# Chriz122/ultralytics_pro

Measured on AMD Instinct MI355X. Metric: images/sec (whole job = n_gpus x per-GPU bs=32) YOLOv8n 640x640 (forward + Detect decode + NMS), higher is better.
Workload: dtype bf16

## Files before the change

include/upa.h:

```cpp
#ifndef UPA_H
#define UPA_H
#include <stddef.h>
#include <stdint.h>

#ifdef __cplusplus
extern "C" {
#endif

enum { UPA_F32 = 0, UPA_BF16 = 1, UPA_U8_BGR_HWC = 2  };
enum { UPA_ACT_NONE = 0, UPA_ACT_SILU = 1, UPA_ACT_RELU = 2 };
enum { UPA_OK = 0, UPA_EINVAL = -1, UPA_EUNSUPPORTED = -2, UPA_EWORKSPACE = -3, UPA_ELAUNCH = -4 };

typedef struct upa_opts {
  uint32_t size;
  int32_t conv_big;
  int32_t conv_big_bm;
  int32_t conv_ckt;
  int32_t no_ws, no_pipe, no_1x1, no_c16, no_upcat;
  int32_t pipe_all;
  int32_t pipe_min_tiles;
  int32_t pipe_wgs, c16_wgs;
  int32_t c1_mt, c1_waves, c1_wgs;
  int32_t pair;
  int32_t pair_tile64, pair_tile32;
  int32_t no_pair_cv2;
  int32_t c2f;
  int32_t c2f16_waves;
  int32_t c2f32_th;
  int32_t no_branch_tail;
  int32_t branch_tail_bm;
  int32_t stem_wgs, stemf_wgs, stemf_waves, stem_no_mfma;
  int32_t ablate_conv, ablate_pipe, ablate_c1, ablate_stem;
  int32_t c2f64_max_px;
  int32_t conv_ws3;
  int32_t no_group;
  int32_t no_c2f32_up;
  int32_t no_xcd;
  int32_t keys_only;
  int32_t conv_p8;
  int32_t c2f_stream;
  int32_t c2f_stream_rows;
  int32_t no_stack_first;
  int32_t no_epi_stats;
  int32_t nms_stages;
  int32_t nms_first_prefix;
  int32_t detect_stream;
  int32_t detect_stream_rows;
  int32_t no_sppf_front;
  int32_t no_c2f16_down;
} upa_opts;

int upa_version(void);
const char* upa_last_error(void);
size_t upa_opts_size(void);

size_t upa_conv_packed_weight_bytes(int cout, int cin, int k, int dtype);
int upa_pack_conv_weight(const float* w_oihw, int cout, int cin, int k, int dtype, void* out);
int upa_conv2d_bias_act(const void* x, int n, int h, int w, int cin, int ldx,
                        const void* w_packed, const float* bias ,
                        void* y, int cout, int ldy,
                        const void* residual , int ldr,
                        int k, int stride, int pad, int act, int dtype, const upa_opts* opts, void* stream);
typedef struct upa_conv_problem {
  const void* x; int32_t n, h, w, cin, ldx;
  const void* w_packed; const float* bias;
  void* y; int32_t cout, ldy;
  const void* residual; int32_t ldr;
} upa_conv_problem;
int upa_conv2d_bias_act_group(const upa_conv_problem* probs, int count, int k, int stride, int pad, int act, int dtype,
                              const upa_opts* opts, void* stream);

int upa_conv2d_pool2(const void* x, int n, int h, int w, int cin, int ldx, const void* w_packed, const float* bias, void* y, int cout,
                     int ldy, int k, int stride, int pad, int act, int dtype, const upa_opts* opts, void* stream);
int upa_conv2d_stem_nchw_pool2(const void* x_nchw, int x_dtype, int n, int cin, int h, int w, const float* w_oihw, const float* bias,
                               void* y, int cout, int ldy, int k, int stride, int pad, int act, int dtype, const upa_opts* opts,
                               void* stream);

int upa_conv_variant(int n, int h, int w, int cin, int cout, int k, int stride, int pad, int dtype, const upa_opts* opts);

int upa_bottleneck_pair(const void* x, int n, int h, int w, int c, int ldx, const void* w1_packed, const float* b1,
                        const void* w2_packed, const float* b2, void* y, int ldy, int residual, int act, int dtype,
                        const upa_opts* opts, void* stream);
int upa_bottleneck_pair_e(const void* x, int n, int h, int w, int c, int cmid, int ldx, const void* w1_packed, const float* b1,
                          const void* w2_packed, const float* b2, void* y, int ldy, int residual, int act, int dtype,
                          const upa_opts* opts, void* stream);


size_t upa_stem_packed_weight_bytes(int cout, int cin, int k);
int upa_pack_stem_weight(const float* w_oihw, int cout, int cin, int k, float* out );
int upa_conv2d_stem_nchw(const void* x_nchw, int x_dtype, int n, int cin, int h, int w,
                         const float* w_oihw, const float* bias, void* y, int cout, int ldy,
                         int k, int stride, int pad, int act, int dtype, const upa_opts* opts, void* stream);

int upa_stem_conv_fused(const void* x, int n, int h, int w, const float* w0, const float* b0, const void* w1,
                        const float* b1, void* y, int ldy, const upa_opts* opts, void* stream);
int upa_stem_conv_fused_k(const void* x, int n, int h, int w, int k0, const float* w0, const float* b0, const void* w1,
                          const float* b1, void* y, int ldy, const upa_opts* opts, void* stream);
int upa_stem_conv_fused_c(const void* x, int n, int h, int w, int k0, int c0, const float* w0, const float* b0, const void* w1,
                          const float* b1, void* y, int ldy, const upa_opts* opts, void* stream);
int upa_stem_conv_fused_s(const void* x, int n, int h, int w, int k0, int s0, int c0, const float* w0, const float* b0,
                          const void* w1, const float* b1, void* y, int ldy, const upa_opts* opts, void* stream);

// ... 227 lines not shown
```

ultralytics_pro_amd/_lib.py:

```python

from __future__ import annotations

import ctypes as C
import os
from pathlib import Path

import torch

UPA_F32, UPA_BF16, UPA_U8_BGR_HWC = 0, 1, 2
UPA_EUNSUPPORTED = -2
ACT_NONE, ACT_SILU, ACT_RELU = 0, 1, 2

_PKG = Path(__file__).resolve().parent
LIB_PATH = Path(os.environ.get("UPA_HIP_LIB", _PKG / "libupa_hip.so"))

_vp, _i, _f, _sz = C.c_void_p, C.c_int, C.c_float, C.c_size_t


class Opts(C.Structure):

    _fields_ = [("size", C.c_uint32), ("conv_big", _i), ("conv_big_bm", _i), ("conv_ckt", _i),
                ("no_ws", _i), ("no_pipe", _i), ("no_1x1", _i), ("no_c16", _i), ("no_upcat", _i),
                ("pipe_all", _i), ("pipe_min_tiles", _i), ("pipe_wgs", _i), ("c16_wgs", _i),
                ("c1_mt", _i), ("c1_waves", _i), ("c1_wgs", _i),
                ("pair", _i), ("pair_tile64", _i), ("pair_tile32", _i), ("no_pair_cv2", _i),
                ("c2f", _i), ("c2f16_waves", _i), ("c2f32_th", _i),
                ("no_branch_tail", _i), ("branch_tail_bm", _i),
                ("stem_wgs", _i), ("stemf_wgs", _i), ("stemf_waves", _i), ("stem_no_mfma", _i),
                ("ablate_conv", _i), ("ablate_pipe", _i), ("ablate_c1", _i), ("ablate_stem", _i), ("c2f64_max_px", _i), ("conv_ws3", _i), ("no_group", _i), ("no_c2f32_up", _i), ("no_xcd", _i), ("keys_only", _i), ("conv_p8", _i), ("c2f_stream", _i), ("c2f_stream_rows", _i), ("no_stack_first", _i), ("no_epi_stats", _i), ("nms_stages", _i), ("nms_first_prefix", _i), ("detect_stream", _i), ("detect_stream_rows", _i), ("no_sppf_front", _i), ("no_c2f16_down", _i)]

    def __init__(self, **kw):
        super().__init__()
        self.size = C.sizeof(Opts)
        for k, v in kw.items():
            if k in dict(self._fields_):
                setattr(self, k, int(v))
            else:
                raise AttributeError(f"upa_opts has no field '{k}'")

    def replace(self, **kw) -> "Opts":
        o = Opts()
        C.memmove(C.byref(o), C.byref(self), C.sizeof(Opts))
        for k, v in kw.items():
            setattr(o, k, int(v))
        return o

    _ENV = {"UPA_CONV_BIG": ("conv_big", lambda v: {0: 1, 1: 0, 2: 2}[int(v)]), "UPA_CONV_BIG_BM": ("conv_big_bm", int), "UPA_CONV_WS3": ("conv_ws3", int),
            "UPA_CONV_CKT": ("conv_ckt", int), "UPA_CONV_NO_WS": ("no_ws", lambda v: 1), "UPA_CONV_NO_PIPE": ("no_pipe", lambda v: 1),
            "UPA_CONV_NO_1X1": ("no_1x1", lambda v: 1), "UPA_CONV_NO_C16": ("no_c16", lambda v: 1), "UPA_NO_UPCAT": ("no_upcat", lambda v: 1),
            "UPA_PIPE_ALL": ("pipe_all", lambda v: 1), "UPA_PIPE_MIN_TILES": ("pipe_min_tiles", int), "UPA_PIPE_WGS": ("pipe_wgs", int),
            "UPA_C16_WGS": ("c16_wgs", int), "UPA_C1_MT": ("c1_mt", int), "UPA_C1_WAVES": ("c1_waves", int), "UPA_C1_WGS": ("c1_wgs", int),
            "UPA_NO_PAIR": ("pair", lambda v: {0: 2, 1: 1, 2: 0, 3: 3}[int(v)]), "UPA_PAIR_T64": ("pair_tile64", int),
            "UPA_PAIR_T32": ("pair_tile32", int), "UPA_NO_PAIR_CV2": ("no_pair_cv2", int), "UPA_NO_C2F": ("c2f", int),
            "UPA_C2F16_WAVES": ("c2f16_waves", int), "UPA_C2F32_TH": ("c2f32_th", int), "UPA_NO_BRANCH_TAIL": ("no_branch_tail", int),
            "UPA_BRANCH_TAIL_BM": ("branch_tail_bm", int), "UPA_STEM_WGS": ("stem_wgs", int), "UPA_STEMF_WGS": ("stemf_wgs", int),
            "UPA_STEMF_WAVES": ("stemf_waves", int), "UPA_STEM_NO_MFMA": ("stem_no_mfma", lambda v: 1),
            "UPA_CONV_ABLATE": ("ablate_conv", int), "UPA_PIPE_ABLATE": ("ablate_pipe", int), "UPA_C1_ABLATE": ("ablate_c1", int),
            "UPA_STEM_ABLATE": ("ablate_stem", int)}

    @classmethod
    def from_env(cls, env=None) -> "Opts":
        env = os.environ if env is None else env
        o = cls()
        for name, (field, conv) in cls._ENV.items():
            if name in env:
                setattr(o, field, conv(env[name]))
        return o


class BranchLevel(C.Structure):
    _fields_ = [("x", C.c_void_p), ("n", _i), ("h", _i), ("w", _i), ("c", _i), ("ldx", _i), ("w3_packed", C.c_void_p), ("b3", C.c_void_p),
                ("wt_packed", C.c_void_p), ("bt", C.c_void_p), ("stride_px", C.c_float), ("a0", _i)]


class DetectBranch(C.Structure):
    _fields_ = [("c", _i), ("reserved", _i), ("w1", C.c_void_p), ("b1", C.c_void_p), ("w2", C.c_void_p), ("b2", C.c_void_p),
                ("wt", C.c_void_p), ("bt", C.c_void_p)]


class ConvProblem(C.Structure):
    _fields_ = [("x", C.c_void_p), ("n", _i), ("h", _i), ("w", _i), ("cin", _i), ("ldx", _i), ("w_packed", C.c_void_p), ("bias", C.c_void_p),
                ("y", C.c_void_p), ("cout", _i), ("ldy", _i), ("residual", C.c_void_p), ("ldr", _i)]
# ... 169 lines not shown
```

ultralytics_pro_amd/csrc/conv_big.hip:

```cpp
#include <stdlib.h>

#include <mutex>
#include <type_traits>
#include <unordered_map>

#include "common.h"
#include "conv_pipe.h"
UPA_STAMP_DEFINE(conv_big)

template <int KS, int STRIDE, int WM, int WN, int MT, int NT, int TAIL = 0>
__device__ __forceinline__ void conv_big_body(const BigParams& p, const int bid0) {
  static_assert(WM * WN == 8, "8 waves per workgroup");
  static_assert(TAIL == 0 || TAIL == 3 || TAIL == 4 || WN == 1, "a tail needs every channel of a pixel in one wave");
  static_assert(TAIL != 1 || (NT % 2) == 0, "box branch: 64 channels");
  static_assert(TAIL != 3 || (NT % 2) == 0, "the statistics epilogue pairs n-tiles");
  static_assert(TAIL != 4 || ((NT % 2) == 0 && KS == 2 && STRIDE == 1), "the interleaving epilogue: 2 x 2 phase kernels, paired n-tiles");
  constexpr int NTB = WN * NT;
  constexpr int WBUF = 2 * NTB * 1024;
  extern __shared__ __attribute__((aligned(16))) char smem[];
  const int tid = threadIdx.x;
  const int lane = tid & 63;
  const int wave = __builtin_amdgcn_readfirstlane(tid >> 6);
  const int r = lane & 15, g = lane >> 4;
  const int wm = wave / WN, wn = wave % WN;

  const int tilesPerImg = p.tilesX * p.tilesY;
  int bid = p.no_xcd ? bid0 : upa_xcd_tile(bid0, tilesPerImg * p.N);
  const int n = bid / tilesPerImg;
  bid -= n * tilesPerImg;
  const int tyi = bid / p.tilesX;
  const int txi = bid - tyi * p.tilesX;
  const int oy0 = tyi * p.TH, ox0 = txi * p.TW;
  const int iy0 = oy0 * STRIDE - p.pad, ix0 = ox0 * STRIDE - p.pad;
  const int ntb0 = blockIdx.y * NTB;

  const int haloItems = p.IH * p.IWp * 8;
  const int haloPadded = (haloItems + 63) & ~63;
  char* hal = smem;
  char* wbuf = smem + (size_t)haloPadded * 16;

  int pl0[MT], pty[MT], ptx[MT];
#pragma unroll
  for (int i = 0; i < MT; ++i) {
    const int pp = (wm * MT + i) * 16 + r;
    int ty = (int)__umulhi((unsigned)pp, p.magicTW);
    int tx = pp - ty * p.TW;
    if (ty >= p.TH) { ty = p.TH; tx = 0; }
    pty[i] = ty;
    ptx[i] = tx;
    pl0[i] = ty < p.TH ? (ty * STRIDE) * p.IWp + tx : 0;
  }

  f32x4 acc[MT][NT];
#pragma unroll
  for (int i = 0; i < MT; ++i)
#pragma unroll
    for (int j = 0; j < NT; ++j) acc[i][j] = f32x4{0.f, 0.f, 0.f, 0.f};

  constexpr int TAPS = KS * KS;
  const int nChunks = (p.KTT + 1) >> 1;

  auto stage_halo = [&](int c) __attribute__((always_inline)) {
    const int c0 = c * 64;
    for (int base = wave * 64; base < haloPadded; base += 512) {
      const int idx = base + lane;
      const int pix = idx >> 3;
      const int slot = idx & 7;
      const int cg = slot ^ (pix & 7);
      const int py = (int)__umulhi((unsigned)pix, p.magicIW);
      const int qx = pix - py * p.IWp;
      int px = qx;
      if constexpr (STRIDE == 2) px = qx < p.HALF ? 2 * qx : 2 * (qx - p.HALF) + 1;
      const int iy = iy0 + py, ix = ix0 + px;
      const int ch = c0 + cg * 8;
      const char* src = reinterpret_cast<const char*>(g_zero16);
      if (idx < haloItems && px < p.IW && iy >= 0 && iy < p.H && ix >= 0 && ix < p.W && ch < p.Cin)
        src = p.x + ((((size_t)n * p.H + iy) * p.W + ix) * (size_t)p.ldx + ch) * 2;
      lds_dma16(src, hal + base * 16);
    }
  };
  auto stage_w = [&](int c, int tap, int b) __attribute__((always_inline)) {
#pragma unroll
    for (int f0 = 0; f0 < 2 * NTB; f0 += 8) {
      const int f = f0 + wave;
      if (f < 2 * NTB) {
        const int kt = f / NTB, j = f - kt * NTB;
        const int ktg = c * 2 + kt;
        const int nt = ntb0 + j;
        const char* src = reinterpret_cast<const char*>(g_zero16);
        if (ktg < p.KTT && nt < p.NTn) src = p.w + (((size_t)(tap * p.KTT + ktg) * p.NTn + nt) * 64 + lane) * 16;
        lds_dma16(src, wbuf + b * WBUF + f * 1024);
      }
    }
  };

  UPA_STAMP_AT(0);
  UPA_STAMP_HWID();
  stage_halo(0);
  stage_w(0, 0, 0);
  int buf = 0;
  for (int c = 0; c < nChunks; ++c) {
    int kh = 0, kw = 0;
#pragma unroll 1
    for (int tap = 0; tap < TAPS; ++tap) {
      asm volatile("s_waitcnt vmcnt(0)" ::: "memory");
      __syncthreads();
      if (c == 0) UPA_STAMP_AT(1 + tap);
      if (tap + 1 < TAPS) stage_w(c, tap + 1, buf ^ 1);
      const int tapshift = kh * p.IWp + (STRIDE == 2 ? (kw >> 1) + (kw & 1) * p.HALF : kw);
      const char* wb = wbuf + buf * WBUF + (wn * NT) * 1024 + lane * 16;
      int paddr[MT], pswz[MT];
#pragma unroll
      for (int i = 0; i < MT; ++i) {
        const int pl = pl0[i] + tapshift;
        paddr[i] = pl * 128;
        pswz[i] = pl & 7;
      }
#pragma unroll
      for (int kt = 0; kt < 2; ++kt) {
        if constexpr (TAIL == 2) {
          if (kt == 1 && c * 2 + 1 >= p.KTT) break;
        }
        if constexpr (NT <= 6) {
          u32x4 a[NT], b[MT];
#pragma unroll
          for (int j = 0; j < NT; ++j) a[j] = *reinterpret_cast<const u32x4*>(wb + (kt * NTB + j) * 1024);
#pragma unroll
          for (int i = 0; i < MT; ++i) b[i] = *reinterpret_cast<const u32x4*>(hal + paddr[i] + (((kt * 4 + g) ^ pswz[i]) << 4));
#pragma unroll
          for (int i = 0; i < MT; ++i)
#pragma unroll
            for (int j = 0; j < NT; ++j)
              acc[i][j] = __builtin_amdgcn_mfma_f32_16x16x32_bf16(*reinterpret_cast<const bf16x8*>(&a[j]),
                                                                  *reinterpret_cast<const bf16x8*>(&b[i]), acc[i][j], 0, 0, 0);
        } else {
          constexpr int GS = (NT + 1) / 2;
          u32x4 b[MT];
#pragma unroll
          for (int i = 0; i < MT; ++i) b[i] = *reinterpret_cast<const u32x4*>(hal + paddr[i] + (((kt * 4 + g) ^ pswz[i]) << 4));
#pragma unroll
          for (int j0 = 0; j0 < NT; j0 += GS) {
            u32x4 a[GS];
#pragma unroll
            for (int j = 0; j < GS; ++j)
              if (j0 + j < NT) a[j] = *reinterpret_cast<const u32x4*>(wb + (kt * NTB + j0 + j) * 1024);
#pragma unroll
            for (int i = 0; i < MT; ++i)
#pragma unroll
              for (int j = 0; j < GS; ++j)
                if (j0 + j < NT)
                  acc[i][j0 + j] = __builtin_amdgcn_mfma_f32_16x16x32_bf16(*reinterpret_cast<const bf16x8*>(&a[j]),
                                                                           *reinterpret_cast<const bf16x8*>(&b[i]), acc[i][j0 + j], 0, 0, 0);
            __builtin_amdgcn_sched_barrier(0);
          }
        }
      }
      buf ^= 1;
      if (++kw == KS) { kw = 0; ++kh; }
    }
    if (c + 1 < nChunks) {
      __syncthreads();
      stage_halo(c + 1);
      stage_w(c + 1, 0, buf);
    }
  }
  UPA_STAMP_AT(10);

  if constexpr (TAIL == 1 || TAIL == 2) {
    f32x4 bv[NT];
#pragma unroll
    for (int j = 0; j < NT; ++j) bv[j] = *reinterpret_cast<const f32x4*>(p.bias + j * 16 + g * 4);
    f32x4 acc2[MT][NT];
#pragma unroll
    for (int i = 0; i < MT; ++i)
#pragma unroll
      for (int j = 0; j < NT; ++j) acc2[i][j] = f32x4{0.f, 0.f, 0.f, 0.f};
#pragma unroll
    for (int s2 = 0; s2 < NT / 2; ++s2) {
      u32x4 hb[MT];
#pragma unroll
      for (int i = 0; i < MT; ++i) {
        float v0[4], v1[4];
#pragma unroll
        for (int q = 0; q < 4; ++q) {
          v0[q] = act_rcp<UPA_ACT_SILU>(acc[i][2 * s2][q] + bv[2 * s2][q]);
          v1[q] = act_rcp<UPA_ACT_SILU>(acc[i][2 * s2 + 1][q] + bv[2 * s2 + 1][q]);
        }
        hb[i] = u32x4{pack_bf16x2(v0[0], v0[1]), pack_bf16x2(v0[2], v0[3]), pack_bf16x2(v1[0], v1[1]), pack_bf16x2(v1[2], v1[3])};
      }
#pragma unroll
      for (int j = 0; j < NT; ++j) {
        const u32x4 a2 = *reinterpret_cast<const u32x4*>(p.tw + ((size_t)(s2 * NT + j) * 64 + lane) * 16);
#pragma unroll
        for (int i = 0; i < MT; ++i)
          acc2[i][j] = __builtin_amdgcn_mfma_f32_16x16x32_bf16(*reinterpret_cast<const bf16x8*>(&a2),
                                                               *reinterpret_cast<const bf16x8*>(&hb[i]), acc2[i][j], 0, 0, 0);
      }
    }
    if constexpr (NT & 1) {
      typedef __attribute__((ext_vector_type(4))) short s16x4;
      constexpr int j0 = NT - 1, s2 = NT / 2;
      u32x2 hh[MT];
#pragma unroll
      for (int i = 0; i < MT; ++i) {
        float v0[4];
#pragma unroll
        for (int q = 0; q < 4; ++q) v0[q] = act_rcp<UPA_ACT_SILU>(acc[i][j0][q] + bv[j0][q]);
        hh[i] = u32x2{pack_bf16x2(v0[0], v0[1]), pack_bf16x2(v0[2], v0[3])};
      }
#pragma unroll
      for (int j = 0; j < NT; ++j) {
        const u32x2 a2 = *reinterpret_cast<const u32x2*>(p.tw + ((size_t)(s2 * NT + j) * 64 + lane) * 16);
#pragma unroll
        for (int i = 0; i < MT; ++i)
          acc2[i][j] = __builtin_amdgcn_mfma_f32_16x16x16bf16_1k(*reinterpret_cast<const s16x4*>(&a2),
                                                                 *reinterpret_cast<const s16x4*>(&hh[i]), acc2[i][j], 0, 0, 0);
// ... 181 lines not shown
  else if (p.act == UPA_ACT_RELU) epilogue(std::integral_constant<int, UPA_ACT_RELU>{});
  else epilogue(std::integral_constant<int, UPA_ACT_NONE>{});
  UPA_STAMP_AT(11);
#ifdef UPA_STAMP
  asm volatile("s_waitcnt vmcnt(0)" ::: "memory");
  UPA_STAMP_AT(12);
#endif
}

template <int KS, int STRIDE, int WM, int WN, int MT, int NT, int TAIL = 0>
__global__ __launch_bounds__(512, 4) void conv_big_kernel(const BigParams p) {
  conv_big_body<KS, STRIDE, WM, WN, MT, NT, TAIL>(p, (int)blockIdx.x);
}

template <int KS, int STRIDE, int WM, int WN, int MT, int NT, int TAIL = 0>
__global__ __launch_bounds__(512, 4) void conv_big_pair_kernel(const BigParams p0, const BigParams p1, const int split) {
  if ((int)blockIdx.x < split) conv_big_body<KS, STRIDE, WM, WN, MT, NT, TAIL>(p0, (int)blockIdx.x);
  else conv_big_body<KS, STRIDE, WM, WN, MT, NT, TAIL>(p1, (int)blockIdx.x - split);
}
template <int KS, int STRIDE, int WM, int WN, int MT, int NT, int TAIL = 0>
__global__ __launch_bounds__(512, 4) void conv_big_tri_kernel(const BigParams p0, const BigParams p1, const BigParams p2, const int s0,
                                                              const int s1) {
  if ((int)blockIdx.x < s0) conv_big_body<KS, STRIDE, WM, WN, MT, NT, TAIL>(p0, (int)blockIdx.x);
  else if ((int)blockIdx.x < s1) conv_big_body<KS, STRIDE, WM, WN, MT, NT, TAIL>(p1, (int)blockIdx.x - s0);
  else conv_big_body<KS, STRIDE, WM, WN, MT, NT, TAIL>(p2, (int)blockIdx.x - s1);
}

template <int KS_, int STRIDE_, int WM_, int WN_, int MT_, int NT_, int TAIL_>
struct BigCfg {
  static constexpr int NTB = WN_ * NT_;
  __device__ static __forceinline__ void run(const BigParams& p, int bid) { conv_big_body<KS_, STRIDE_, WM_, WN_, MT_, NT_, TAIL_>(p, bid); }
};
template <class CA, class CB>
__global__ __launch_bounds__(512, 4) void conv_big_mix_kernel(const BigParams a0, const BigParams a1, const BigParams b0, const BigParams b1,
                                                              const int s0, const int s1, const int s2) {
  const int b = (int)blockIdx.x;
  if (b < s0) CA::run(a0, b);
  else if (b < s1) CA::run(a1, b - s0);
  else if (b < s2) CB::run(b0, b - s1);
  else CB::run(b1, b - s2);
}

namespace {
void big_halo_geometry(BigParams& p, bool tight = false) {
  p.IH = (p.TH - 1) * p.stride + p.KS;
  p.IW = (p.TW - 1) * p.stride + p.KS;
  p.HALF = p.stride == 2 ? (p.IW + 1) / 2 : 0;
  const int minp = p.stride == 2 ? 2 * p.HALF : p.IW;
  p.IWp = tight ? minp : upa_lds_pick_pitch(minp, p.TW, p.TH * p.TW, p.stride);
  p.magicTW = (unsigned)((0x100000000ULL + p.TW - 1) / p.TW);
  p.magicIW = (unsigned)((0x100000000ULL + p.IWp - 1) / p.IWp);
}
size_t big_halo_bytes(const BigParams& p) { return (((size_t)p.IH * p.IWp * 8 + 63) & ~(size_t)63) * 16; }

bool big_pick_tile(BigParams& p, int bm, int ntb, size_t lds_cap) {
  struct Pick { int th, tw, tight; };
  static std::mutex mu;
  static std::unordered_map<unsigned long long, Pick> memo;
  const unsigned long long key = ((unsigned long long)p.OH << 48) ^ ((unsigned long long)p.OW << 32) ^ ((unsigned long long)bm << 20) ^
                                 ((unsigned long long)ntb << 12) ^ ((unsigned long long)(lds_cap >> 9) << 3) ^ ((unsigned long long)p.KS << 56) ^ (p.KS == 3 ? 4u : 0u) ^
                                 (p.stride == 2 ? 2u : 0u);
  {
    std::lock_guard<std::mutex> lk(mu);
    auto it = memo.find(key);
    if (it != memo.end()) {
      if (it->second.th <= 0) return false;
      p.TH = it->second.th; p.TW = it->second.tw;
      big_halo_geometry(p, it->second.tight != 0);
      return true;
    }
  }
  long best = -1;
  int bth = 0, btw = 0;
  bool btight = false;
  for (int tw = 2; tw <= 256 && tw <= ((p.OW + 1) & ~1); ++tw) {
    int th0 = bm / tw;
    if (th0 > p.OH) th0 = p.OH;
    if (th0 < 1) continue;
    const int thb = cdiv(p.OH, cdiv(p.OH, th0));
    for (int pass = 0; pass < 2; ++pass) {
      const int th = pass ? thb : th0;
      if (pass && thb == th0) break;
      for (int tight = 0; tight < 2; ++tight) {
        p.TH = th; p.TW = tw;
        big_halo_geometry(p, tight != 0);
        const size_t lds = big_halo_bytes(p) + 2 * (size_t)(2 * ntb * 1024) + 256;
        if (lds > lds_cap) continue;
        const long tiles = (long)cdiv(p.OW, tw) * cdiv(p.OH, th);
        const long cost = tiles * 65536 + (long)p.IH * p.IWp;
        if (best < 0 || cost < best) { best = cost; bth = th; btw = tw; btight = tight != 0; }
        break;
      }
    }
  }
  p.TH = bth; p.TW = btw;
  if (best >= 0) big_halo_geometry(p, btight);
  {
    std::lock_guard<std::mutex> lk(mu);
    memo[key] = Pick{best >= 0 ? bth : 0, btw, btight ? 1 : 0};
  }
  return best >= 0;
}

template <int KS, int STRIDE, int WM, int WN, int MT, int NT, int TAIL = 0>
int big_launch_inst(const BigParams& p, size_t lds, hipStream_t s) {
  constexpr int NTB = WN * NT;
// ... 76 lines not shown
  return (unsigned short)(u >> 16);
}

extern "C" int upa_pack_tail_weight(const float* w, int cout, int cin, void* out) {
  UPA_CHECK_ARG(w && out && cout > 0 && cin > 0, "pack_tail_weight: bad args");
  const int ks = cdiv(cin, 32), nt = cdiv(cout, 16);
  unsigned short* o = (unsigned short*)out;
  size_t idx = 0;
  for (int s = 0; s < ks; ++s)
    for (int j = 0; j < nt; ++j)
      for (int lane = 0; lane < 64; ++lane) {
        const int g = lane >> 4, r = lane & 15;
        const int co = 16 * j + r;
        for (int e = 0; e < 8; ++e, ++idx) {
          const int ci = 32 * s + (e < 4 ? 4 * g + e : 16 + 4 * g + e - 4);
          o[idx] = big_host_bf16((co < cout && ci < cin) ? w[(size_t)co * cin + ci] : 0.f);
        }
      }
  return UPA_OK;
}

namespace {
int branch_tail_prepare(BigParams& p, int& ntb, int& bm, size_t& lds, const void* x, int n, int h, int w, int c, int ldx,
                        const void* w3_packed, const float* b3, const void* wt_packed, const float* bt, int kind, int nc,
                        float stride_px, float* y, int a_total, int a0, unsigned long long* best_keys, int dtype, const upa_opts* opts) {
  UPA_CHECK_ARG(x && w3_packed && b3 && wt_packed && bt && y, "detect_branch_tail: null pointer");
  UPA_CHECK_ARG(kind == 1 || kind == 2, "detect_branch_tail: kind must be 1 (box) or 2 (class)");
  UPA_CHECK_ARG(n > 0 && h > 0 && w > 0 && a0 >= 0 && a0 + h * w <= a_total, "detect_branch_tail: level does not fit a_total");
  const int off = UPA_OPT(opts, no_branch_tail);
  ntb = kind == 1 ? 4 : (c == 80 ? 5 : 6);
  if (off || dtype != UPA_BF16 || c % 8 != 0 || ldx % 8 != 0 || h * w < 2 || w < 2 || (kind == 1 && c != 64) ||
      (kind == 2 && (c > 96 || nc > ntb * 16)) || ((uintptr_t)x % 16) != 0 || !upa_magic_exact((long)h * w - 1, w)) {
    upa_set_error("detect_branch_tail: outside the fused form (bf16; box c = 64; class c <= 96, nc <= 96)");
    return UPA_EUNSUPPORTED;
  }
  memset(&p, 0, sizeof(p));
  p.x = (const char*)x; p.w = (const char*)w3_packed; p.bias = b3; p.tw = (const char*)wt_packed; p.tb = bt;
  p.N = n; p.H = h; p.W = w; p.Cin = c; p.ldx = ldx; p.OH = h; p.OW = w; p.Cout = ntb * 16; p.KS = 3; p.stride = 1; p.pad = 1;
  p.act = UPA_ACT_SILU;
  p.KTT = cdiv(c, 32);
  p.NTn = ntb;
  p.de.y = y; p.de.a_total = a_total; p.de.a0 = a0; p.de.HW = h * w; p.de.W = w;
  p.de.magicHW = upa_magic_div(h * w); p.de.magicW = upa_magic_div(w);
  p.de.nc = nc; p.de.stride_px = stride_px;
  if (kind == 2 && best_keys && (long)a_total * nc < (1L << 31)) p.de.best_keys = best_keys;
  p.de.keys_only = (p.de.best_keys && UPA_OPT(opts, keys_only)) ? 1 : 0;
  p.no_xcd = UPA_OPT(opts, no_xcd);
  const long px = (long)n * h * w;
  bm = (px + 255) / 256 < upa_num_cus() ? 128 : 256;
  if (const int f = UPA_OPT(opts, branch_tail_bm); f == 128 || f == 256) bm = f;
  if (!big_pick_tile(p, bm, ntb, 80 * 1024 - 512) && !big_pick_tile(p, bm, ntb, 160 * 1024)) return UPA_EUNSUPPORTED;
  p.tilesX = cdiv(p.OW, p.TW);
  p.tilesY = cdiv(p.OH, p.TH);
  lds = big_halo_bytes(p) + 2 * (size_t)(2 * ntb * 1024) + 256;
  return UPA_OK;
}
int branch_tail_launch(const BigParams& p, int kind, int ntb, int bm, size_t lds, hipStream_t s) {
  if (kind == 1) return bm == 256 ? big_launch_inst<3, 1, 8, 1, 2, 4, 1>(p, lds, s) : big_launch_inst<3, 1, 8, 1, 1, 4, 1>(p, lds, s);
  if (ntb == 5) return bm == 256 ? big_launch_inst<3, 1, 8, 1, 2, 5, 2>(p, lds, s) : big_launch_inst<3, 1, 8, 1, 1, 5, 2>(p, lds, s);
  return bm == 256 ? big_launch_inst<3, 1, 8, 1, 2, 6, 2>(p, lds, s) : big_launch_inst<3, 1, 8, 1, 1, 6, 2>(p, lds, s);
}
}

extern "C" int upa_detect_branch_tail(const void* x, int n, int h, int w, int c, int ldx, const void* w3_packed, const float* b3,
                                      const void* wt_packed, const float* bt, int kind, int nc, float stride_px, float* y,
                                      int a_total, int a0, unsigned long long* best_keys, int dtype, const upa_opts* opts,
                                      void* stream) {
  BigParams p;
  int ntb = 0, bm = 0;
  size_t lds = 0;
  if (const int rc = branch_tail_prepare(p, ntb, bm, lds, x, n, h, w, c, ldx, w3_packed, b3, wt_packed, bt, kind, nc, stride_px, y,
                                         a_total, a0, best_keys, dtype, opts); rc != UPA_OK)
    return rc;
  return branch_tail_launch(p, kind, ntb, bm, lds, (hipStream_t)stream);
}

extern "C" int upa_detect_branch_tail_group(const upa_branch_level* levels, int count, int kind, int nc, float* y, int a_total,
                                            unsigned long long* best_keys, int dtype, const upa_opts* opts, void* stream) {
  UPA_CHECK_ARG(levels && count >= 1 && count <= 8, "detect_branch_tail_group: 1..8 levels");
  BigParams ps[8];
  int ntb[8], bm[8];
  size_t lds[8];
  for (int i = 0; i < count; ++i) {
    const upa_branch_level& v = levels[i];
    if (const int rc = branch_tail_prepare(ps[i], ntb[i], bm[i], lds[i], v.x, v.n, v.h, v.w, v.c, v.ldx, v.w3_packed, v.b3, v.wt_packed,
                                           v.bt, kind, nc, v.stride_px, y, a_total, v.a0, best_keys, dtype, opts); rc != UPA_OK)
      return rc;
  }
  hipStream_t s = (hipStream_t)stream;
  const int grouping = UPA_OPT(opts, no_group);
  auto max3 = [](size_t a, size_t b, size_t c) { return a > b ? (a > c ? a : c) : (b > c ? b : c); };
  for (int i = 0; i < count;) {
    if (grouping == 2 && i + 2 < count && ntb[i] == ntb[i + 1] && ntb[i] == ntb[i + 2] && ntb[i] != 6 && bm[i + 1] == 128 && bm[i + 2] == 128) {
      BigParams p0 = ps[i];
      int ntb0 = ntb[i], bm0 = bm[i];
      size_t lds0 = lds[i];
      int rc = UPA_OK;
      if (bm0 != 128) {
        upa_opts o;
        memset(&o, 0, sizeof(o));
        if (opts) memcpy(&o, opts, opts->size < sizeof(o) ? opts->size : sizeof(o));
        o.size = sizeof(o);
        o.branch_tail_bm = 128;
        const upa_branch_level& v = levels[i];
        rc = branch_tail_prepare(p0, ntb0, bm0, lds0, v.x, v.n, v.h, v.w, v.c, v.ldx, v.w3_packed, v.b3, v.wt_packed, v.bt, kind, nc,
                                 v.stride_px, y, a_total, v.a0, best_keys, dtype, &o);
      }
// ... 63 lines not shown
  return UPA_OK;
}

bool upa_conv_big_pick_tile(BigParams& p, int bm, int ntb, size_t lds_cap) { return big_pick_tile(p, bm, ntb, lds_cap); }

bool upa_conv_big_eligible(const ConvShape& s, const upa_opts* opts) {
  const int mode = UPA_OPT(opts, conv_big);
  if (mode == 1) return false;
  const int k = s.k, stride = s.stride, cin = s.cin, cout = s.cout;
  if (s.dtype != UPA_BF16 || !((k == 1 && stride == 1) || (k == 2 && stride == 1) || (k == 3 && (stride == 1 || stride == 2))) || s.pad != k / 2) return false;
  if (cin % 8 != 0 || s.ldx % 8 != 0 || cout % 8 != 0 || s.ldy % 8 != 0 || s.ldr % 8 != 0) return false;
  if (s.act != UPA_ACT_SILU && s.act != UPA_ACT_NONE && s.act != UPA_ACT_RELU) return false;
  if (mode == 2) return cout >= 64;
  const int oh = (s.h + 2 * s.pad - k) / stride + 1, ow = (s.w + 2 * s.pad - k) / stride + 1;
  const long px = (long)s.n * oh * ow;
  if (k == 1) {
    if (cout % 128 != 0 || px < 2048) return false;
    if (cout >= 1024 && cin >= 128 && px >= 32 * 1024) return true;
    return cin >= 512 && !upa_conv1x1_eligible(s, opts);
  }
  if (cin < 64 || px < 2048) return false;
  if (cout % 128 == 0) return cin >= 128 || (px >= 8192 && (stride == 2 || px >= 200 * 1024));
  if (px < 8192) return false;
  if (cout == 80 || cout == 96) return stride == 1 && k == 3;
  if (cout == 144) return stride == 1 && k == 3;
  if (cout == 64) return stride == 1;
  return false;
}

namespace {
int big_prepare(BigParams& p, int& ntb, int& bm, size_t& lds, const upa_opts* opts, bool query_only, int force_ntb = 0) {
  p.KTT = (p.Cin + 31) / 32;
  p.NTn = (p.Cout + 15) / 16;
  ntb = p.NTn <= 4 ? 4 : (p.NTn <= 6 ? 6 : 8);
  if (p.NTn == 5 && p.KS == 3 && p.stride == 1) ntb = 5;
  if (p.NTn == 9 && p.KS == 3 && p.stride == 1) ntb = 9;
  if (force_ntb == 5 && p.NTn <= 5 && p.KS == 3 && p.stride == 1) ntb = 5;
  const long px = (long)p.N * p.OH * p.OW;
  if (ntb == 8 && p.NTn % 4 == 0 && (px + 127) / 128 * cdiv(p.NTn, 8) < upa_num_cus()) ntb = 4;
  const int cols = cdiv(p.NTn, ntb);
  bm = 256;
  if ((px + 255) / 256 * cols < upa_num_cus()) bm = 128;
  if (const int f = UPA_OPT(opts, conv_big_bm); f == 128 || f == 256 || (f == 512 && p.KS == 3 && p.stride == 1 && (ntb == 4 || ntb == 5))) bm = f;
  if (query_only) return UPA_OK;
  if (p.KS == 1) {
    p.N = 1; p.H = 1; p.W = (int)px; p.OH = 1; p.OW = (int)px;
    p.TH = 1; p.TW = bm;
    big_halo_geometry(p, true);
  } else if (!big_pick_tile(p, bm, ntb, 80 * 1024 - 512) && !big_pick_tile(p, bm, ntb, 160 * 1024)) {
    return UPA_EUNSUPPORTED;
  }
  p.tilesX = cdiv(p.OW, p.TW);
  p.tilesY = cdiv(p.OH, p.TH);
  lds = big_halo_bytes(p) + 2 * (size_t)(2 * ntb * 1024) + 256;
  if (lds > 160 * 1024) return UPA_EUNSUPPORTED;
  return UPA_OK;
}
template <int WM, int WN, int MT, int NT>
int big_launch_ks_stats(const BigParams& p, size_t lds, hipStream_t s) {
  if (p.KS == 1) return big_launch_inst<1, 1, WM, WN, MT, NT, 3>(p, lds, s);
  if (p.KS != 3) return UPA_EUNSUPPORTED;
  if (p.stride == 2) return big_launch_inst<3, 2, WM, WN, MT, NT, 3>(p, lds, s);
  return big_launch_inst<3, 1, WM, WN, MT, NT, 3>(p, lds, s);
}
int big_dispatch_stats(const BigParams& p, int ntb, int bm, size_t lds, hipStream_t s) {
  if (bm != 128 && bm != 256) return UPA_EUNSUPPORTED;
  if (ntb == 8) return bm == 256 ? big_launch_ks_stats<4, 2, 4, 4>(p, lds, s) : big_launch_ks_stats<4, 2, 2, 4>(p, lds, s);
  if (ntb == 4) return bm == 256 ? big_launch_ks_stats<8, 1, 2, 4>(p, lds, s) : big_launch_ks_stats<4, 2, 2, 2>(p, lds, s);
  return UPA_EUNSUPPORTED;
}
int big_dispatch(const BigParams& p, int ntb, int bm, size_t lds, hipStream_t s) {
  if (bm == 512) return ntb == 5 ? big_launch_inst<3, 1, 8, 1, 4, 5>(p, lds, s) : big_launch_inst<3, 1, 8, 1, 4, 4>(p, lds, s);
  if (ntb == 5) return bm == 256 ? big_launch_inst<3, 1, 8, 1, 2, 5>(p, lds, s) : big_launch_inst<3, 1, 8, 1, 1, 5>(p, lds, s);
  if (ntb == 9) return bm == 256 ? big_launch_inst<3, 1, 8, 1, 2, 9>(p, lds, s) : big_launch_inst<3, 1, 8, 1, 1, 9>(p, lds, s);
  if (ntb == 8) return bm == 256 ? big_launch_ks<4, 2, 4, 4>(p, lds, s) : big_launch_ks<4, 2, 2, 4>(p, lds, s);
  if (ntb == 6) return bm == 256 ? big_launch_ks<4, 2, 4, 3>(p, lds, s) : big_launch_ks<4, 2, 2, 3>(p, lds, s);
  return bm == 256 ? big_launch_ks<8, 1, 2, 4>(p, lds, s) : big_launch_ks<4, 2, 2, 2>(p, lds, s);
}
}

int upa_conv_big_launch(BigParams p, int query_only, int* variant, void* stream, const upa_opts* opts) {
  p.no_xcd = UPA_OPT(opts, no_xcd);
  int ntb = 0, bm = 0;
  size_t lds = 0;
  const int rc = big_prepare(p, ntb, bm, lds, opts, query_only != 0);
  if (variant) *variant = (1 << 23) | (ntb << 4) | (bm >> 7);
  if (query_only || rc != UPA_OK) return rc;
  return big_dispatch(p, ntb, bm, lds, (hipStream_t)stream);
}

int upa_conv_big_launch_interleave(BigParams p, void* stream, const upa_opts* opts) {
  p.no_xcd = UPA_OPT(opts, no_xcd);
  if (p.KS != 2 || p.stride != 1 || p.act != UPA_ACT_NONE || p.bias || p.il_c % 8 != 0 || p.Cout != 4 * p.il_c) return UPA_EUNSUPPORTED;
  int ntb = 0, bm = 0;
  size_t lds = 0;
  if (const int rc = big_prepare(p, ntb, bm, lds, opts, false); rc != UPA_OK) return rc;
  if (ntb != 8 || (bm != 128 && bm != 256)) return UPA_EUNSUPPORTED;
  hipStream_t s = (hipStream_t)stream;
  return bm == 256 ? big_launch_inst<2, 1, 4, 2, 4, 4, 4>(p, lds, s) : big_launch_inst<2, 1, 4, 2, 2, 4, 4>(p, lds, s);
}

int upa_conv_big_launch_stats(BigParams p, int* rows, long max_rows, void* stream, const upa_opts* opts) {
  p.no_xcd = UPA_OPT(opts, no_xcd);
  if (!p.stats || p.res || p.act != UPA_ACT_NONE) return UPA_EUNSUPPORTED;
  int ntb = 0, bm = 0;
  size_t lds = 0;
  if (const int rc = big_prepare(p, ntb, bm, lds, opts, false); rc != UPA_OK) return rc;
// ... 81 lines not shown
```

ultralytics_pro_amd/csrc/conv_pipe.h:

```cpp
#pragma once
struct ConvShape {
  int n, h, w, cin, ldx, cout, ldy, ldr, k, stride, pad, act, dtype;
};
struct PipeParams {
  const char* x;
  char* y;
  const char* res;
  const char* w;
  const float* bias;
  int N, H, W, Cin, ldx, Cout, ldy, ldr;
  int KTT, NTn, nt0;
  int tilesX, tilesY, numTiles;
  int act;
  int pool;
#ifdef UPA_ABLATE
  int ablate;
#endif
};
bool upa_conv_pipe_eligible(const ConvShape& s, const upa_opts* opts);
int upa_conv_pipe_launch(PipeParams p, int query_only, int* variant, void* stream, const upa_opts* opts);

#include "detect_epi.h"
struct C1Params {
  const char* x;
  char* y;
  const char* w;
  const float* bias;
  int P;
  int Cin, ldx, Cout, ldy;
  int KTT, NTn, groups;
  int act;
#ifdef UPA_ABLATE
  int ablate;
#endif
  int epi;
  DetectEpi de;
  float* stats;
  int stats_ld;
  const char* up;
  int upKT, up_ld, upH, upW;
  unsigned upMagicW, upMagicH;
};
bool upa_conv1x1_eligible(const ConvShape& s, const upa_opts* opts);
int upa_conv1x1_launch(C1Params p, int n_pixels, int query_only, int* variant, void* stream, const upa_opts* opts);
int upa_conv1x1_launch_stats(C1Params p, int n_pixels, int* rows, long max_rows, void* stream, const upa_opts* opts);

struct BigParams {
  const char* x;
  char* y;
  const char* res;
  const char* w;
  const float* bias;
  int N, H, W, Cin, ldx, OH, OW, Cout, ldy, ldr;
  int KS, stride, pad;
  int TH, TW, tilesX, tilesY, IH, IW;
  int IWp;
  int HALF;
  int KTT, NTn;
  int act;
  unsigned magicTW, magicIW;
  int no_xcd;
  const char* tw;
  const float* tb;
  DetectEpi de;
  float* stats;
  int stats_ld;
  int il_h, il_w, il_c;
};
bool upa_conv_big_eligible(const ConvShape& s, const upa_opts* opts);
int upa_conv_big_launch(BigParams p, int query_only, int* variant, void* stream, const upa_opts* opts);
int upa_conv_big_launch_stats(BigParams p, int* rows, long max_rows, void* stream, const upa_opts* opts);
int upa_conv_big_launch_interleave(BigParams p, void* stream, const upa_opts* opts);
int upa_conv_big_launch_group(const BigParams* probs, int count, int* consumed, void* stream, const upa_opts* opts);

bool upa_conv_big_pick_tile(BigParams& p, int bm, int ntb, size_t lds_cap);

bool upa_conv_p8_eligible(const ConvShape& s, const upa_opts* opts);
int upa_conv_p8_launch(BigParams p, int query_only, int* variant, void* stream, const upa_opts* opts);

bool upa_conv_ws3_eligible(const ConvShape& s, const upa_opts* opts);
int upa_conv_ws3_launch(BigParams p, int query_only, int* variant, void* stream, const upa_opts* opts);
int upa_conv_ws3_launch_stats(BigParams p, int* rows, long max_rows, void* stream, const upa_opts* opts);

struct PairParams {
  const char* x;
  char* y;
  const char* w1;
  const char* w2;
  const float* b1;
  const float* b2;
  int N, H, W, OH, OW, ldx, ldy;
  int TH, TW, tilesX, tilesY;
  int IWp, MWp;
  unsigned magicIW, magicMW, magicTW;
  const char* y0;
  const char* wc_std;
  const char* wc_b;
  const float* bc;
  char* out; int ldout;
};
```

Before: 61100.

## Add opt-in cross-chunk halo prefetch and multi-stage LDS ring to big conv

Adds a double-buffered halo for conv kernels with KS>1. The next channel chunk's halo is staged piece by piece during the current chunk's taps, with partial vmcnt waits. Adds a 2–3 stage LDS ring for 1x1 kernels with BM=128, so that halo and weight loads for later chunks overlap MFMA work. The aim is to remove the full-drain barrier and serial halo reload between chunks, at the cost of more LDS per workgroup and possibly lower occupancy. Both paths are chosen through a new no_chunk_prefetch option, and the default value appears to keep the old plain layout.

```diff
diff --git a/include/upa.h b/include/upa.h
--- a/include/upa.h
+++ b/include/upa.h
@@ -48,6 +48,7 @@
   int32_t detect_stream_rows;
   int32_t no_sppf_front;
   int32_t no_c2f16_down;
+  int32_t no_chunk_prefetch;
 } upa_opts;
 
 int upa_version(void);
diff --git a/ultralytics_pro_amd/_lib.py b/ultralytics_pro_amd/_lib.py
--- a/ultralytics_pro_amd/_lib.py
+++ b/ultralytics_pro_amd/_lib.py
@@ -27,7 +27,8 @@
                 ("c2f", _i), ("c2f16_waves", _i), ("c2f32_th", _i),
                 ("no_branch_tail", _i), ("branch_tail_bm", _i),
                 ("stem_wgs", _i), ("stemf_wgs", _i), ("stemf_waves", _i), ("stem_no_mfma", _i),
-                ("ablate_conv", _i), ("ablate_pipe", _i), ("ablate_c1", _i), ("ablate_stem", _i), ("c2f64_max_px", _i), ("conv_ws3", _i), ("no_group", _i), ("no_c2f32_up", _i), ("no_xcd", _i), ("keys_only", _i), ("conv_p8", _i), ("c2f_stream", _i), ("c2f_stream_rows", _i), ("no_stack_first", _i), ("no_epi_stats", _i), ("nms_stages", _i), ("nms_first_prefix", _i), ("detect_stream", _i), ("detect_stream_rows", _i), ("no_sppf_front", _i), ("no_c2f16_down", _i)]
+                ("ablate_conv", _i), ("ablate_pipe", _i), ("ablate_c1", _i), ("ablate_stem", _i), ("c2f64_max_px", _i), ("conv_ws3", _i), ("no_group", _i), ("no_c2f32_up", _i), ("no_xcd", _i), ("keys_only", _i), ("conv_p8", _i), ("c2f_stream", _i), ("c2f_stream_rows", _i), ("no_stack_first", _i), ("no_epi_stats", _i), ("nms_stages", _i), ("nms_first_prefix", _i), ("detect_stream", _i), ("detect_stream_rows", _i), ("no_sppf_front", _i), ("no_c2f16_down", _i),
+                ("no_chunk_prefetch", _i)]
 
     def __init__(self, **kw):
         super().__init__()
diff --git a/ultralytics_pro_amd/csrc/conv_big.hip b/ultralytics_pro_amd/csrc/conv_big.hip
--- a/ultralytics_pro_amd/csrc/conv_big.hip
+++ b/ultralytics_pro_amd/csrc/conv_big.hip
@@ -7,6 +7,33 @@
 #include "common.h"
 #include "conv_pipe.h"
 UPA_STAMP_DEFINE(conv_big)
+
+namespace {
+template <int N>
+__device__ __forceinline__ void big_vm_wait_imm() {
+  static_assert(N >= 0 && N < 64, "vmcnt is a 6-bit field");
+  asm volatile("s_waitcnt vmcnt(%0)" ::"n"(N) : "memory");
+}
+template <int NS>
+__device__ __forceinline__ void big_vm_wait_stages(const int young) {
+  if (young == 1) big_vm_wait_imm<NS>();
+  else if (young == 2) big_vm_wait_imm<2 * NS>();
+  else big_vm_wait_imm<0>();
+}
+__device__ __forceinline__ void big_vm_wait_piece(const int n) {
+  if (n == 1) big_vm_wait_imm<1>();
+  else if (n == 2) big_vm_wait_imm<2>();
+  else if (n == 3) big_vm_wait_imm<3>();
+  else big_vm_wait_imm<0>();
+}
+__device__ __forceinline__ void big_barrier() {
+  __builtin_amdgcn_sched_barrier(0);
+  asm volatile("s_waitcnt lgkmcnt(0)" ::: "memory");
+  __builtin_amdgcn_s_barrier();
+  asm volatile("" ::: "memory");
+  __builtin_amdgcn_sched_barrier(0);
+}
+}
 
 template <int KS, int STRIDE, int WM, int WN, int MT, int NT, int TAIL = 0>
 __device__ __forceinline__ void conv_big_body(const BigParams& p, const int bid0) {
@@ -36,8 +63,11 @@
 
   const int haloItems = p.IH * p.IWp * 8;
   const int haloPadded = (haloItems + 63) & ~63;
-  char* hal = smem;
-  char* wbuf = smem + (size_t)haloPadded * 16;
+  const int HB = haloPadded * 16;
+  constexpr int BM = WM * MT * 16;
+  constexpr bool RING_OK = KS == 1 && BM == 128, HALO2_OK = KS > 1 && BM <= 256;
+  const bool halo2 = HALO2_OK && p.halo2 != 0;
+  char* wbuf = smem + (halo2 ? 2 * HB : HB);
 
   int pl0[MT], pty[MT], ptx[MT];
 #pragma unroll
@@ -60,9 +90,11 @@
   constexpr int TAPS = KS * KS;
   const int nChunks = (p.KTT + 1) >> 1;
 
-  auto stage_halo = [&](int c) __attribute__((always_inline)) {
+  auto stage_halo = [&](int c, char* dst, int k0, int kstep) __attribute__((always_inline)) {
     const int c0 = c * 64;
-    for (int base = wave * 64; base < haloPadded; base += 512) {
+    int issued = 0;
+    for (int base = wave * 64 + k0 * 512; base < haloPadded; base += kstep * 512) {
+      ++issued;
       const int idx = base + lane;
       const int pix = idx >> 3;
       const int slot = idx & 7;
@@ -76,10 +108,11 @@
       const char* src = reinterpret_cast<const char*>(g_zero16);
       if (idx < haloItems && px < p.IW && iy >= 0 && iy < p.H && ix >= 0 && ix < p.W && ch < p.Cin)
         src = p.x + ((((size_t)n * p.H + iy) * p.W + ix) * (size_t)p.ldx + ch) * 2;
-      lds_dma16(src, hal + base * 16);
-    }
+      lds_dma16(src, dst + base * 16);
+    }
+    return issued;
   };
-  auto stage_w = [&](int c, int tap, int b) __attribute__((always_inline)) {
+  auto stage_w = [&](int c, int tap, char* dst) __attribute__((always_inline)) {
 #pragma unroll
     for (int f0 = 0; f0 < 2 * NTB; f0 += 8) {
       const int f = f0 + wave;
@@ -89,79 +122,129 @@
         const int nt = ntb0 + j;
         const char* src = reinterpret_cast<const char*>(g_zero16);
         if (ktg < p.KTT && nt < p.NTn) src = p.w + (((size_t)(tap * p.KTT + ktg) * p.NTn + nt) * 64 + lane) * 16;
-        lds_dma16(src, wbuf + b * WBUF + f * 1024);
+        lds_dma16(src, dst + f * 1024);
+      }
+    }
+  };
+
+  auto mma_tap = [&](const char* hb, const char* wslab, const int tapshift, const int c) __attribute__((always_inline)) {
+    const char* wb = wslab + (wn * NT) * 1024 + lane * 16;
+    int paddr[MT], pswz[MT];
+#pragma unroll
+    for (int i = 0; i < MT; ++i) {
+      const int pl = pl0[i] + tapshift;
+      paddr[i] = pl * 128;
+      pswz[i] = pl & 7;
+    }
+#pragma unroll
+    for (int kt = 0; kt < 2; ++kt) {
+      if constexpr (TAIL == 2) {
+        if (kt == 1 && c * 2 + 1 >= p.KTT) break;
+      }
+      if constexpr (NT <= 6) {
+        u32x4 a[NT], b[MT];
+#pragma unroll
+        for (int j = 0; j < NT; ++j) a[j] = *reinterpret_cast<const u32x4*>(wb + (kt * NTB + j) * 1024);
+#pragma unroll
+        for (int i = 0; i < MT; ++i) b[i] = *reinterpret_cast<const u32x4*>(hb + paddr[i] + (((kt * 4 + g) ^ pswz[i]) << 4));
+#pragma unroll
+        for (int i = 0; i < MT; ++i)
+#pragma unroll
+          for (int j = 0; j < NT; ++j)
+            acc[i][j] = __builtin_amdgcn_mfma_f32_16x16x32_bf16(*reinterpret_cast<const bf16x8*>(&a[j]),
+                                                                *reinterpret_cast<const bf16x8*>(&b[i]), acc[i][j], 0, 0, 0);
+      } else {
+        constexpr int GS = (NT + 1) / 2;
+        u32x4 b[MT];
+#pragma unroll
+        for (int i = 0; i < MT; ++i) b[i] = *reinterpret_cast<const u32x4*>(hb + paddr[i] + (((kt * 4 + g) ^ pswz[i]) << 4));
+#pragma unroll
+        for (int j0 = 0; j0 < NT; j0 += GS) {
+          u32x4 a[GS];
+#pragma unroll
+          for (int j = 0; j < GS; ++j)
+            if (j0 + j < NT) a[j] = *reinterpret_cast<const u32x4*>(wb + (kt * NTB + j0 + j) * 1024);
+#pragma unroll
+          for (int i = 0; i < MT; ++i)
+#pragma unroll
+            for (int j = 0; j < GS; ++j)
+              if (j0 + j < NT)
+                acc[i][j0 + j] = __builtin_amdgcn_mfma_f32_16x16x32_bf16(*reinterpret_cast<const bf16x8*>(&a[j]),
+                                                                         *reinterpret_cast<const bf16x8*>(&b[i]), acc[i][j0 + j], 0, 0, 0);
+          __builtin_amdgcn_sched_barrier(0);
+        }
       }
     }
   };
 
   UPA_STAMP_AT(0);
   UPA_STAMP_HWID();
-  stage_halo(0);
-  stage_w(0, 0, 0);
-  int buf = 0;
-  for (int c = 0; c < nChunks; ++c) {
-    int kh = 0, kw = 0;
+  bool ringed = false;
+  if constexpr (RING_OK) {
+    if (p.ring >= 2) {
+      ringed = true;
+      constexpr int HPW = WM * MT / 4;
+      constexpr int NWLO = (2 * NTB) / 8, NWHI = (2 * NTB + 7) / 8;
+      const int nw = (2 * NTB - wave + 7) >> 3;
+      const int D = p.ring;
+      const int STG = HB + WBUF;
+      auto stage = [&](int c, char* dst) __attribute__((always_inline)) {
+#pragma unroll
+        for (int k = 0; k < HPW; ++k) stage_halo(c, dst, k, HPW);
+        stage_w(c, 0, dst + HB);
+      };
+      for (int d = 0; d < D; ++d) stage(d, smem + d * STG);
+      char* cur = smem;
+      char* prev = smem;
+      for (int c = 0; c < nChunks; ++c) {
+        int young = D - 1;
+        if (c > 0) young = (c + D - 2 < nChunks - 1 ? c + D - 2 : nChunks - 1) - c;
+        if (NWLO == NWHI || nw == NWHI) big_vm_wait_stages<HPW + NWHI>(young);
+        else big_vm_wait_stages<HPW + NWLO>(young);
+        big_barrier();
+        if (c < 9) UPA_STAMP_AT(1 + c);
+        if (c > 0 && c + D - 1 < nChunks) stage(c + D - 1, prev);
+        mma_tap(cur, cur + HB, 0, c);
+        prev = cur;
+        cur += STG;
+        if (cur == smem + D * STG) cur = smem;
+      }
+    }
+  }
+  if (!ringed) {
+    stage_halo(0, smem, 0, 1);
+    stage_w(0, 0, wbuf);
+    int buf = 0;
+    int young = 0;
+    for (int c = 0; c < nChunks; ++c) {
+      const bool pre = halo2 && c + 1 < nChunks;
+      const char* hcur = smem + ((halo2 && (c & 1)) ? HB : 0);
+      char* hnext = smem + ((c & 1) ? 0 : HB);
+      int kh = 0, kw = 0;
 #pragma unroll 1
-    for (int tap = 0; tap < TAPS; ++tap) {
-      asm volatile("s_waitcnt vmcnt(0)" ::: "memory");
-      __syncthreads();
-      if (c == 0) UPA_STAMP_AT(1 + tap);
-      if (tap + 1 < TAPS) stage_w(c, tap + 1, buf ^ 1);
-      const int tapshift = kh * p.IWp + (STRIDE == 2 ? (kw >> 1) + (kw & 1) * p.HALF : kw);
-      const char* wb = wbuf + buf * WBUF + (wn * NT) * 1024 + lane * 16;
-      int paddr[MT], pswz[MT];
-#pragma unroll
-      for (int i = 0; i < MT; ++i) {
-        const int pl = pl0[i] + tapshift;
-        paddr[i] = pl * 128;
-        pswz[i] = pl & 7;
-      }
-#pragma unroll
-      for (int kt = 0; kt < 2; ++kt) {
-        if constexpr (TAIL == 2) {
-          if (kt == 1 && c * 2 + 1 >= p.KTT) break;
+      for (int tap = 0; tap < TAPS; ++tap) {
+        if (halo2) {
+          big_vm_wait_piece(young);
+          big_barrier();
+        } else {
+          asm volatile("s_waitcnt vmcnt(0)" ::: "memory");
+          __syncthreads();
         }
-        if constexpr (NT <= 6) {
-          u32x4 a[NT], b[MT];
-#pragma unroll
-          for (int j = 0; j < NT; ++j) a[j] = *reinterpret_cast<const u32x4*>(wb + (kt * NTB + j) * 1024);
-#pragma unroll
-          for (int i = 0; i < MT; ++i) b[i] = *reinterpret_cast<const u32x4*>(hal + paddr[i] + (((kt * 4 + g) ^ pswz[i]) << 4));
-#pragma unroll
-          for (int i = 0; i < MT; ++i)
-#pragma unroll
-            for (int j = 0; j < NT; ++j)
-              acc[i][j] = __builtin_amdgcn_mfma_f32_16x16x32_bf16(*reinterpret_cast<const bf16x8*>(&a[j]),
-                                                                  *reinterpret_cast<const bf16x8*>(&b[i]), acc[i][j], 0, 0, 0);
-        } else {
-          constexpr int GS = (NT + 1) / 2;
-          u32x4 b[MT];
-#pragma unroll
-          for (int i = 0; i < MT; ++i) b[i] = *reinterpret_cast<const u32x4*>(hal + paddr[i] + (((kt * 4 + g) ^ pswz[i]) << 4));
-#pragma unroll
-          for (int j0 = 0; j0 < NT; j0 += GS) {
-            u32x4 a[GS];
-#pragma unroll
-            for (int j = 0; j < GS; ++j)
-              if (j0 + j < NT) a[j] = *reinterpret_cast<const u32x4*>(wb + (kt * NTB + j0 + j) * 1024);
-#pragma unroll
-            for (int i = 0; i < MT; ++i)
-#pragma unroll
-              for (int j = 0; j < GS; ++j)
-                if (j0 + j < NT)
-                  acc[i][j0 + j] = __builtin_amdgcn_mfma_f32_16x16x32_bf16(*reinterpret_cast<const bf16x8*>(&a[j]),
-                                                                           *reinterpret_cast<const bf16x8*>(&b[i]), acc[i][j0 + j], 0, 0, 0);
-            __builtin_amdgcn_sched_barrier(0);
-          }
-        }
-      }
-      buf ^= 1;
-      if (++kw == KS) { kw = 0; ++kh; }
-    }
-    if (c + 1 < nChunks) {
-      __syncthreads();
-      stage_halo(c + 1);
-      stage_w(c + 1, 0, buf);
+        if (KS == 1 ? c < 9 : c == 0) UPA_STAMP_AT(1 + (KS == 1 ? c : tap));
+        if (tap + 1 < TAPS) stage_w(c, tap + 1, wbuf + (buf ^ 1) * WBUF);
+        else if (pre) stage_w(c + 1, 0, wbuf + (buf ^ 1) * WBUF);
+        young = pre ? stage_halo(c + 1, hnext, tap, TAPS) : 0;
+        const int tapshift = kh * p.IWp + (STRIDE == 2 ? (kw >> 1) + (kw & 1) * p.HALF : kw);
+        mma_tap(hcur, wbuf + buf * WBUF, tapshift, c);
+        buf ^= 1;
+        if (++kw == KS) { kw = 0; ++kh; }
+      }
+      young = 0;
+      if (!halo2 && c + 1 < nChunks) {
+        __syncthreads();
+        stage_halo(c + 1, smem, 0, 1);
+        stage_w(c + 1, 0, wbuf + buf * WBUF);
+      }
     }
   }
   UPA_STAMP_AT(10);
@@ -449,6 +532,31 @@
   p.magicIW = (unsigned)((0x100000000ULL + p.IWp - 1) / p.IWp);
 }
 size_t big_halo_bytes(const BigParams& p) { return (((size_t)p.IH * p.IWp * 8 + 63) & ~(size_t)63) * 16; }
+
+size_t big_plan_lds(BigParams& p, int ntb, int bm, const upa_opts* opts) {
+  const size_t hb = big_halo_bytes(p), wb = (size_t)2 * ntb * 1024;
+  const size_t plain = hb + 2 * wb + 256;
+  p.ring = 0;
+  p.halo2 = 0;
+  const int sw = UPA_OPT(opts, no_chunk_prefetch);
+  if (sw == 0 || sw == 1) return plain;
+  const int chunks = (p.KTT + 1) / 2;
+  const size_t cap = plain <= 80 * 1024 - 512 ? 80 * 1024 - 512 : 160 * 1024;
+  if (p.KS == 1) {
+    if (sw == 2) return plain;
+    long d = (long)((cap - 256) / (hb + wb));
+    if (d > (sw == 4 ? 2 : 3)) d = sw == 4 ? 2 : 3;
+    if (d > chunks) d = chunks;
+    if (d >= 2 && p.IH == 1 && p.IWp == p.TW && p.TW == bm && bm == 128) {
+      p.ring = (int)d;
+      return (size_t)d * (hb + wb) + 256;
+    }
+  } else if (sw != 3 && sw != 4 && chunks >= 2 && plain + hb <= cap && bm <= 256) {
+    p.halo2 = 1;
+    return plain + hb;
+  }
+  return plain;
+}
 
 bool big_pick_tile(BigParams& p, int bm, int ntb, size_t lds_cap) {
   struct Pick { int th, tw, tight; };
@@ -631,7 +739,7 @@
   if (!big_pick_tile(p, bm, ntb, 80 * 1024 - 512) && !big_pick_tile(p, bm, ntb, 160 * 1024)) return UPA_EUNSUPPORTED;
   p.tilesX = cdiv(p.OW, p.TW);
   p.tilesY = cdiv(p.OH, p.TH);
-  lds = big_halo_bytes(p) + 2 * (size_t)(2 * ntb * 1024) + 256;
+  lds = big_plan_lds(p, ntb, bm, opts);
   return UPA_OK;
 }
 int branch_tail_launch(const BigParams& p, int kind, int ntb, int bm, size_t lds, hipStream_t s) {
@@ -801,7 +909,7 @@
   }
   p.tilesX = cdiv(p.OW, p.TW);
   p.tilesY = cdiv(p.OH, p.TH);
-  lds = big_halo_bytes(p) + 2 * (size_t)(2 * ntb * 1024) + 256;
+  lds = big_plan_lds(p, ntb, bm, opts);
   if (lds > 160 * 1024) return UPA_EUNSUPPORTED;
   return UPA_OK;
 }
diff --git a/ultralytics_pro_amd/csrc/conv_pipe.h b/ultralytics_pro_amd/csrc/conv_pipe.h
--- a/ultralytics_pro_amd/csrc/conv_pipe.h
+++ b/ultralytics_pro_amd/csrc/conv_pipe.h
@@ -66,6 +66,7 @@
   float* stats;
   int stats_ld;
   int il_h, il_w, il_c;
+  int ring, halo2;
 };
 bool upa_conv_big_eligible(const ConvShape& s, const upa_opts* opts);
 int upa_conv_big_launch(BigParams p, int query_only, int* variant, void* stream, const upa_opts* opts);
```

Result: slower. 59710 (-2.3%).
